# kr4b/pigs

Measured on AMD Instinct MI355X. Metric: sample-points/sec (fwd + 1st + 2nd derivatives, fused), higher is better.
Workload: dtype f32; 1 GPU; c3: 65536 Gaussians x 1024x1024 grid, 1024 rows x 1024 points per GPU, d=2, c=1, kappa=0.5, orders 0-2; gaussians=65536, points_per_gpu=1048576, step=preprocess (cold: nothing reused) + fused forward (orders 0..2)

## Files before the change

pigs_amd/csrc/build_choice.h:

```cpp
#pragma once
#include "plan.h"
#include <stddef.h>
#include <string.h>

namespace pigs {

constexpr uint32_t LISTS_SMALL_TILES = 4096;
constexpr int64_t LATTICE_MIN_POINTS = 1 << 12;
constexpr int64_t COARSE_MIN_POINTS = 1 << 17;
constexpr int64_t STAGE_MIN_POINTS = 1 << 19;
constexpr uint32_t TRUST_MIN_BUILDS = 64;
constexpr float STRIP_MAX_COVER = 64.f;
constexpr int64_t STRIP_MIN_GAUSSIANS = 1024;

struct BuildRequest {
    bool do_samples = false, do_plan = false;
    bool plan_ws_clean = false;
    bool no_lookback = false;
    bool build_lists = true;
    int order = 0;
    bool defer_lists = false, fwd_only = false;
    int64_t N = 0, M = 0;
    int c = 1;
    float q_max = 1.f, q_max_b = 1.f;
};

struct BuildEnv {
    int lattice = -1;
    int lattice_trust = -1;
    int samples_order = 0;
    int gauss_strips = -1;
    int bbox_blocks = -1;
    bool no_ahead = false;
};

struct MemoryAnswer {
    bool coarse = false;
    uint32_t rf = 0, axis = 0;
    bool box_ok = false;
    float box[4] = {0.f, 0.f, 0.f, 0.f};
    bool trust = false;
    bool takes_strips = false;
};

enum BuildKernel : uint32_t {
    K_SAMPLES_BBOX, K_PLAN_ZERO, K_PLAN_COUNT, K_PLAN_SCAN, K_PLAN_SCATTER, K_BINSORT_16, K_BINSORT_1,
    K_LISTS_SMALL,
    K_LISTS
};
struct BuildLaunch {
    BuildKernel kernel;
    uint32_t grid, block, lds;
};
struct BuildChoice {
    bool coarse, no_lattice;
    uint32_t rf_hint, bbox_blocks;
    bool fwd_only, ahead, s_scan_in_scatter, sort_in_count, strips, trusted;
    uint32_t s_blocks;
    float q_max_b;
    BuildLaunch launches[7];
    int n = 0;
    void add(BuildKernel k, uint32_t grid, uint32_t block = 256, uint32_t lds = 0) { launches[n++] = BuildLaunch{k, grid, block, lds}; }
};

inline BuildLaunch list_launch(uint32_t ntiles) {
    const bool small = ntiles <= LISTS_SMALL_TILES && LISTS_TPW != 1;
// ... 135 lines not shown
```

pigs_amd/csrc/build_memory.h:

```cpp
#pragma once
#include <hip/hip_runtime.h>
#include <stdint.h>

namespace pigs {

inline bool current_device(int* dev) {
    if (hipGetDevice(dev) == hipSuccess) return true;
    (void)hipGetLastError();
    return false;
}
inline bool stream_capturing(hipStream_t stream) {
    hipStreamCaptureStatus st = hipStreamCaptureStatusNone;
    if (hipStreamIsCapturing(stream, &st) != hipSuccess) { (void)hipGetLastError(); return false; }
    return st != hipStreamCaptureStatusNone;
}

template <class Key, class State, uint32_t WORDS>
struct BuildMemory {
    struct Slot {
        int device = -1;
        Key key{};
        State st{};
        bool pending = false;
        hipEvent_t ev = nullptr;
        uint32_t* host = nullptr;
        uint64_t stamp = 0;
    };
    void (*landed)(Slot&);
    Slot slots[16];
    uint64_t clock = 0;

    void poll(Slot& s) {
        if (!s.pending) return;
        const hipError_t q = hipEventQuery(s.ev);
        (void)hipGetLastError();
        if (q != hipSuccess) return;
        s.pending = false;
        landed(s);
    }
    Slot* peek(int device, const Key& key) {
        for (auto& s : slots)
            if (s.device == device && s.key == key) return &s;
        return nullptr;
    }
    Slot* find(int device, const Key& key, bool create = false) {
        Slot* lru = nullptr;
        for (auto& s : slots) {
            if (s.device == device && s.key == key) { s.stamp = ++clock; return &s; }
            if (!s.pending && (!lru || s.stamp < lru->stamp)) lru = &s;
        }
        if (!create) return nullptr;
        if (!lru) {
            for (auto& s : slots) {
                poll(s);
                if (!s.pending && (!lru || s.stamp < lru->stamp)) lru = &s;
            }
            if (!lru) return nullptr;
        }
        if (lru->ev && lru->device != device) {
            (void)hipEventDestroy(lru->ev);
            lru->ev = nullptr;
        }
        if (!lru->ev && hipEventCreateWithFlags(&lru->ev, hipEventDisableTiming) != hipSuccess) { lru->ev = nullptr; (void)hipGetLastError(); return nullptr; }
        if (!lru->host && hipHostMalloc((void**)&lru->host, WORDS * sizeof(uint32_t), hipHostMallocPortable) != hipSuccess) { lru->host = nullptr; (void)hipGetLastError(); return nullptr; }
        lru->device = device; lru->key = key; lru->st = State{}; lru->pending = false; lru->stamp = ++clock;
        return lru;
    }
    void request(Slot& s, const void* src, hipStream_t stream) {
        if (hipMemcpyAsync(s.host, src, WORDS * sizeof(uint32_t), hipMemcpyDeviceToHost, stream) == hipSuccess &&
            hipEventRecord(s.ev, stream) == hipSuccess)
            s.pending = true;
        (void)hipGetLastError();
    }
};

}
```

pigs_amd/csrc/plan.hip:

```cpp
#include "pair_math.h"
#include "plan.h"
#include "grid_walk.h"
#include "launch.h"
#include "plan_build.h"
#include "plan_lists.h"
#include "plan_forward.h"
#include "plan_backward.h"
#include "build_choice.h"
#include "build_memory.h"
#include <cstdlib>
#include <cstring>
#include <type_traits>
#include <mutex>
#include <unordered_map>

namespace pigs {

static bool samples_supported(int64_t M) { return M >= 1 && M < (1LL << 31) - 64; }
static bool plan_supported(int64_t N, int64_t M, int c) {
    return samples_supported(M) && N >= 1 && c >= 1 && c <= 2 && N < (1LL << LIST_IDX_BITS);
}

static SamplesView make_samples_view(const SamplesLayout& p, const void* sws) {
    const char* b = (const char*)sws;
// ... 75 lines not shown
    if (coarse) {
        a.scounts = (uint32_t*)(b + s.off_hist);
        a.sagg = (unsigned long long*)(b + s.off_hagg);
        a.sstarts = (uint32_t*)(b + s.off_hstarts);
        a.s_scan_blocks = s.h_scan_blocks;
        a.szero = (uint32_t*)(b + s.off_hagg);
        a.s_zero_words = (uint32_t)((s.off_hstarts - s.off_hagg) / 4);
    } else {
        a.scounts = (uint32_t*)(b + s.off_counts);
        a.sagg = (unsigned long long*)(b + s.off_agg);
        a.sstarts = (uint32_t*)(b + s.off_starts);
        a.s_scan_blocks = s.scan_blocks;
        a.szero = a.scounts;
        a.s_zero_words = (uint32_t)((s.off_starts - s.off_counts) / 4);
    }
}

static int samples_order_setting() {
    const char* e = getenv("PIGS_SAMPLES_ORDER");
    return !e ? 0 : !strcmp(e, "ordered") ? 1 : !strcmp(e, "unordered") ? 2 : 0;
}
static uint32_t lists_product_setting() {
    const char* e = getenv("PIGS_LISTS_PRODUCT");
    return e && e[0] == '0' ? 0u : 1u;
}
static BuildEnv build_env() {
    static const char* const bbox = getenv("PIGS_BBOX_BLOCKS");
    static const bool no_ahead = getenv("PIGS_NO_AHEAD") != nullptr;
    BuildEnv env;
    if (const char* e = getenv("PIGS_LATTICE")) env.lattice = e[0] != '0';
    if (const char* e = getenv("PIGS_LATTICE_TRUST")) env.lattice_trust = e[0] == '0' ? 0 : e[0] == '1' ? 1 : -1;
    env.samples_order = samples_order_setting();
    if (const char* e = getenv("PIGS_GAUSS_STRIPS")) env.gauss_strips = e[0] == '1';
    if (bbox) env.bbox_blocks = atoi(bbox) == 512 ? 512 : 256;
    env.no_ahead = no_ahead;
    return env;
}

struct OrderKey {
    int64_t M;
    bool operator==(const OrderKey& o) const { return M == o.M; }
};
struct PointsKey {
    int64_t N, M;
    bool operator==(const PointsKey& o) const { return N == o.N && M == o.M; }
};
using OrderMemory = BuildMemory<OrderKey, OrderState, ORDER_WORDS>;
using PointsMemory = BuildMemory<PointsKey, PointsState, POINTS_WORDS>;
static void order_landed(OrderMemory::Slot& s) { s.st.absorb(s.host); }
static void points_landed(PointsMemory::Slot& s);
static std::mutex g_memory_mu;
static OrderMemory g_order{order_landed};
static PointsMemory g_points{points_landed};
static void points_landed(PointsMemory::Slot& s) {
    if (s.st.absorb(s.host))
        if (auto* o = g_order.find(s.device, OrderKey{s.key.M})) o->st.turn_around();
}

static MemoryAnswer ask_memories(const BuildRequest& r, const BuildEnv& env, hipStream_t stream) {
    MemoryAnswer m;
    const bool points = strips_asked(r, env);
    int dev = 0;
    if ((!r.do_samples && !points) || !current_device(&dev)) return m;
    const bool cap = stream_capturing(stream);
    std::lock_guard<std::mutex> lock(g_memory_mu);
    if (r.do_samples)
        if (auto* o = g_order.find(dev, OrderKey{r.M})) {
            if (!cap) g_order.poll(*o);
            m.coarse = o->st.coarse; m.rf = o->st.rf; m.axis = o->st.axis;
            if (o->st.box_stable) { m.box_ok = true; memcpy(m.box, o->st.box, sizeof(m.box)); }
            m.trust = !cap && o->st.trusts(env.lattice_trust);
        }
    if (points)
        if (auto* h = g_points.find(dev, PointsKey{r.N, r.M})) {
            if (!cap) g_points.poll(*h);
            m.takes_strips = h->st.takes_strips();
        }
    return m;
}

static void note_order(const SamplesLayout& s, const void* sws, hipStream_t stream, bool trusted) {
    if (!trusted && (s.M < 64 || stream_capturing(stream))) return;
    int dev = 0;
    if (!current_device(&dev)) return;
    std::lock_guard<std::mutex> lock(g_memory_mu);
    auto* o = g_order.find(dev, OrderKey{s.M}, !trusted);
    if (!o) return;
    if (trusted) { ++o->st.trusted; return; }
    const uint32_t nth = o->st.builds++;
    if (o->st.rf != 0u) ++o->st.streak;
    if (!o->pending && o->st.copy_due(nth)) g_order.request(*o, (const char*)sws + s.off_params, stream);
}
static void note_points(const PlanLayout& p, const void* ws, hipStream_t stream, bool trusted = false) {
    int dev = 0;
    if (stream_capturing(stream) || !current_device(&dev)) return;
    std::lock_guard<std::mutex> lock(g_memory_mu);
    auto* h = g_points.find(dev, PointsKey{p.N, p.M}, true);
    if (!h) return;
    const uint32_t nth = h->st.builds++;
    if (!h->pending && h->st.copy_due(nth, trusted))
        g_points.request(*h, &((const PlanParams*)((const char*)ws + p.off_params))->n_points, stream);
}

static bool points_unordered(int64_t M, hipStream_t stream) {
    if (const char* e = getenv("PIGS_STAGE")) return e[0] == '1';
    if (M < STAGE_MIN_POINTS) return false;
    if (getenv("PIGS_SAMPLES_ORDER")) return samples_order_setting() == 2;
    int dev = 0;
    if (!current_device(&dev)) return false;
    const bool cap = stream_capturing(stream);
    std::lock_guard<std::mutex> lock(g_memory_mu);
    auto* o = g_order.peek(dev, OrderKey{M});
    if (!o) return false;
    if (!cap) g_order.poll(*o);
    return o->st.coarse;
}
static bool plan_expects_points(int64_t N, int64_t M, hipStream_t stream) {
    int dev = 0;
    if (!current_device(&dev)) return false;
    const bool cap = stream_capturing(stream);
    std::lock_guard<std::mutex> lock(g_memory_mu);
    auto* h = g_points.find(dev, PointsKey{N, M});
    if (!h) return false;
    if (!cap) g_points.poll(*h);
    return h->st.has_points;
}

int samples_order_hint(int64_t M) {
    int dev = 0;
    if (!current_device(&dev)) return -1;
    std::lock_guard<std::mutex> lock(g_memory_mu);
    auto* o = g_order.find(dev, OrderKey{M});
    if (!o) return -1;
    g_order.poll(*o);
// ... 84 lines not shown
    }
    if (small && strips) hipLaunchKernelGGL((plan_lists_kernel<1, true>), grid, block, 0, stream, la);
    else if (small) hipLaunchKernelGGL((plan_lists_kernel<1, false>), grid, block, 0, stream, la);
    else if (strips) hipLaunchKernelGGL((plan_lists_kernel<LISTS_TPW, true>), grid, block, 0, stream, la);
    else hipLaunchKernelGGL((plan_lists_kernel<LISTS_TPW, false>), grid, block, 0, stream, la);
}

static int run_build(const BuildRequest& r, void* sws, size_t sws_bytes, void* ws, size_t ws_bytes, const void* means,
                     const void* conics, const void* values, const void* samples, hipStream_t stream) {
    if (!samples_supported(r.M)) return PIGS_ERR_UNSUPPORTED;
    const SamplesLayout s = make_samples_layout(r.M);
    if (!sws || sws_bytes < s.total_bytes) return PIGS_ERR_WORKSPACE;
    PlanLayout p{};
    if (r.do_plan) {
        if (!plan_supported(r.N, r.M, r.c)) return PIGS_ERR_UNSUPPORTED;
        if (!(r.q_max > 0.f)) return PIGS_ERR_INVALID;
        p = make_plan_layout(r.N, r.M, r.c);
        if (!ws || ws_bytes < p.total_bytes) return PIGS_ERR_WORKSPACE;
    }
    const BuildEnv env = build_env();
    const MemoryAnswer mem = ask_memories(r, env, stream);
    const BuildChoice b = choose_build(r, s, p, env, mem);
    BuildArgs a{};
    a.do_samples = r.do_samples; a.do_plan = r.do_plan; a.no_lookback = r.no_lookback;
    a.zero_gacc = !r.plan_ws_clean;
    fill_samples_args(a, s, sws, samples, b.coarse);
    if (r.do_plan) fill_plan_args(a, p, ws, r.q_max, b.q_max_b, means, conics, values);
    a.no_lattice = b.no_lattice; a.rf_hint = b.rf_hint; a.bbox_blocks = b.bbox_blocks; a.s_blocks = b.s_blocks;
    a.hint_axis = mem.axis;
    memcpy(a.hint_box, mem.box, sizeof(a.hint_box));
    a.fwd_only = b.fwd_only; a.ahead = b.ahead; a.s_scan_in_scatter = b.s_scan_in_scatter; a.sort_in_count = b.sort_in_count;
    a.strips = b.strips; a.trusted = b.trusted;
    const bool lists = r.do_plan && r.build_lists && !r.defer_lists;
    ListArgs la{};
    if (lists) {
        la = make_list_args(p, s, ws, sws, r.q_max, a.q_max);
        if (b.trusted) {
            la.lattice_broken = &a.params->lattice_broken;
            const float rf = (float)a.rf_hint, rs = (float)(r.M / a.rf_hint);
            la.guard_n[0] = a.hint_axis ? rs : rf; la.guard_n[1] = a.hint_axis ? rf : rs;
            la.guard_e[0] = 16.f * (a.hint_box[2] - a.hint_box[0]) * 1.001f;
            la.guard_e[1] = 16.f * (a.hint_box[3] - a.hint_box[1]) * 1.001f;
        }
    }
    clear_hip_error();
    for (int i = 0; i < b.n; ++i) {
        const BuildLaunch& l = b.launches[i];
        const dim3 grid(l.grid), block(l.block);
        switch (l.kernel) {
            case K_SAMPLES_BBOX: hipLaunchKernelGGL(samples_bbox_kernel, grid, block, l.lds, stream, a); break;
            case K_PLAN_ZERO: hipLaunchKernelGGL(plan_zero_kernel, grid, block, l.lds, stream, a); break;
            case K_PLAN_COUNT: hipLaunchKernelGGL(plan_count_kernel, grid, block, l.lds, stream, a); break;
            case K_PLAN_SCAN: hipLaunchKernelGGL(plan_scan_kernel, grid, block, l.lds, stream, a); break;
            case K_PLAN_SCATTER: hipLaunchKernelGGL(plan_scatter_kernel, grid, block, l.lds, stream, a); break;
            case K_BINSORT_16: hipLaunchKernelGGL(samples_binsort_kernel<16>, grid, block, l.lds, stream, a); break;
            case K_BINSORT_1: hipLaunchKernelGGL(samples_binsort_kernel<1>, grid, block, l.lds, stream, a); break;
            case K_LISTS_SMALL:
            case K_LISTS: launch_lists(l, la, stream, b.strips, b.fwd_only); break;
        }
    }
    const int rc = launch_status();
    if (r.do_plan) defer_set(ws, r.build_lists && r.defer_lists && rc == PIGS_OK, r.q_max, a.q_max);
    if (rc != PIGS_OK) return rc;
    if (lists) note_points(p, ws, stream, b.trusted);
    if (b.trusted || (r.do_samples && r.order == 0)) note_order(s, sws, stream, b.trusted);
    return rc;
}

size_t aggregate_grid_bytes(int64_t N) {
    if (!plan_supported(N, N, 1)) return 0;
    return align_up(make_samples_layout(N).total_bytes, 256) + make_plan_layout(N, N, 1).total_bytes;
}

int aggregate_grid_build(void* ws, size_t ws_bytes, int64_t N, float q_grid, const float* means, const float* conics,
                         hipStream_t stream) {
    if (!plan_supported(N, N, 1)) return PIGS_ERR_UNSUPPORTED;
    if (!ws || ws_bytes < aggregate_grid_bytes(N)) return PIGS_ERR_WORKSPACE;
    const size_t sb = align_up(make_samples_layout(N).total_bytes, 256);
    BuildRequest r;
    r.do_samples = r.do_plan = true; r.build_lists = false;
    r.N = r.M = N; r.c = 1; r.q_max = r.q_max_b = q_grid;
    return run_build(r, ws, sb, (char*)ws + sb, ws_bytes - sb, means, conics, means, means, stream);
}

void aggregate_grid_levels(int64_t N, int64_t* info) {
    const PlanLayout p = make_plan_layout(N, N, 1);
    info[0] = (int64_t)(align_up(make_samples_layout(N).total_bytes, 256) + p.off_params + offsetof(PlanParams, level_mask));
    info[1] = p.L;
}

PlanView aggregate_grid_view(void* ws, int64_t N, float q_grid) {
    const size_t sb = align_up(make_samples_layout(N).total_bytes, 256);
    return make_view(make_plan_layout(N, N, 1), (char*)ws + sb, q_grid);
}

int samples_build(void* sws, size_t sws_bytes, int64_t M, const void* samples, hipStream_t stream) {
    BuildRequest r;
// ... 112 lines not shown
        default: break;
    }
    if constexpr (C == 2) {
        switch (mask) {
            PIGS_CASE(ORDV) PIGS_CASE(ORDC) PIGS_CASE(ORDN)
            default: break;
        }
    }
#undef PIGS_CASE
    if (!done) return PIGS_ERR_UNSUPPORTED;
    hipLaunchKernelGGL((plan_unpermute_kernel<C>), dim3((pv.N + 255) / 256), dim3(256), 0, stream, pv, (float*)a.g_means,
                       (float*)a.g_conics, (float*)a.g_values);
    return launch_status();
}

int plan_forward(void* ws, size_t ws_bytes, const void* sws, size_t sws_bytes, float q_max, const SampleArgs& a,
                 hipStream_t stream) {
    if (!plan_supported(a.N, a.M, a.c)) return PIGS_ERR_UNSUPPORTED;
    const PlanLayout p = make_plan_layout(a.N, a.M, a.c);
    const SamplesLayout s = make_samples_layout(a.M);
    if (!ws || ws_bytes < p.total_bytes || !sws || sws_bytes < s.total_bytes) return PIGS_ERR_WORKSPACE;
    const PlanView pv = make_view(p, ws, q_max);
    const SamplesView sv = make_samples_view(s, sws);
    float* o[4];
    for (int k = 0; k < 4; ++k) o[k] = mask_uses_slot(a.orders_mask, k) ? (float*)a.out[k] : nullptr;
    const int cm = covering_mask_of(a.orders_mask);
    if (a.c != 1 && a.c != 2) return PIGS_ERR_UNSUPPORTED;
    DeferredLists d{};
    ListArgs la{};
    const bool first = defer_take(ws, d);
    if (first) la = make_list_args(p, s, ws, sws, d.q_f, d.q_wide);
    const int rc = a.c == 1 ? plan_forward_c<1>(pv, sv, cm, o, a, stream, first ? &la : nullptr)
                            : plan_forward_c<2>(pv, sv, cm, o, a, stream, first ? &la : nullptr);
    if (first && rc == PIGS_OK) note_points(p, ws, stream);
    return rc;
}

int plan_backward(void* ws, size_t ws_bytes, const void* sws, size_t sws_bytes, float q_max, const SampleArgs& a,
                  hipStream_t stream) {
    if (!plan_supported(a.N, a.M, a.c)) return PIGS_ERR_UNSUPPORTED;
    const PlanLayout p = make_plan_layout(a.N, a.M, a.c);
    const SamplesLayout s = make_samples_layout(a.M);
    if (!ws || ws_bytes < p.total_bytes || !sws || sws_bytes < s.total_bytes) return PIGS_ERR_WORKSPACE;
    const PlanView pv = make_view(p, ws, q_max);
    const SamplesView sv = make_samples_view(s, sws);
    {
        DeferredLists d{};
        if (defer_take(ws, d)) {
            clear_hip_error();
            launch_lists(list_launch(s.ntiles), make_list_args(p, s, ws, sws, d.q_f, d.q_wide), stream);
            const int rc = launch_status();
            if (rc != PIGS_OK) return rc;
            note_points(p, ws, stream);
        }
    }
    const float* g[4];
    for (int k = 0; k < 4; ++k) g[k] = mask_uses_slot(a.orders_mask, k) ? (const float*)a.gout[k] : nullptr;
    const int cm = covering_mask_of(a.orders_mask);
    switch (a.c) {
        case 1: return plan_backward_c<1>(pv, sv, cm, g, a, stream);
        case 2: return plan_backward_c<2>(pv, sv, cm, g, a, stream);
    }
    return PIGS_ERR_UNSUPPORTED;
}

}
```

pigs_amd/csrc/plan_build.h:

```cpp
#pragma once
#include "pair_math.h"
#include "plan.h"
#include "grid_walk.h"
#include <type_traits>

namespace pigs {

struct BuildArgs {
    SampleParams* sparams;
    float4* sboxes;
    float4* slat;
    int no_lattice;
    uint32_t rf_hint;
    uint32_t* scounts;
    unsigned long long* sagg;
    uint32_t* sstarts;
    uint2* skey;
    SPoint* spts;
    const float* samples;
    uint32_t M, scells_cap, s_scan_blocks, s_zero_words;
    uint32_t s_blocks;
    uint32_t* szero;
    int coarse;
    uint32_t cells_per_bin, h_chunk, h_wgs;
// ... 244 lines not shown
#pragma unroll
        for (int k = 0; k < 8; ++k) sh[wave][k] = v[k];
    }
    __syncthreads();
#pragma unroll
    for (int k = 0; k < 8; ++k) {
        float r = sh[0][k];
        for (int w = 1; w < 4; ++w) r = (k & 2) || k >= 4 ? fmaxf(r, sh[w][k]) : fminf(r, sh[w][k]);
        sbox[k] = r;
    }
}
__device__ __forceinline__ bool lattice_compact(const float* sbox, uint32_t rf, uint32_t rs, uint32_t axis) {
    if (rf == 0u) return false;
    const float ex = sbox[2] - sbox[0], ey = sbox[3] - sbox[1];
    const float nx = (float)(axis ? rs : rf), ny = (float)(axis ? rf : rs);
    return 7.f * (sbox[4] + sbox[6]) * nx <= 16.f * ex && 7.f * (sbox[5] + sbox[7]) * ny <= 16.f * ey;
}

struct Run { int start; uint32_t len; bool leader; };
__device__ __forceinline__ Run run_of(uint32_t k, int lane) {
    const uint32_t prev = __shfl_up(k, 1);
    Run r;
    r.leader = lane == 0 || k != prev;
    const uint64_t lm = __ballot(r.leader);
    const uint64_t upto = (2ull << lane) - 1ull;
    r.start = 63 - __builtin_clzll(lm & upto);
    const uint64_t above = lm & ~upto;
    r.len = (uint32_t)((above ? __builtin_ctzll(above) : 64) - lane);
    return r;
}

__device__ __forceinline__ void samples_hist_part(const BuildArgs& a, uint32_t w, const SampleGrid& sg, uint32_t* lh, int lane);

struct GaussLoad { float m[2], c[3]; };
__device__ __forceinline__ void gauss_scatter_one(const BuildArgs& a, uint32_t i, uint32_t pos) {
    float v[2] = {0.f, 0.f};
    for (int k = 0; k < a.c; ++k) v[k] = a.values[(size_t)i * a.c + k];
    a.rec[2 * pos] = make_float4(a.means[2 * i], a.means[2 * i + 1], a.conics[3 * i], a.conics[3 * i + 1]);
    a.rec[2 * pos + 1] = make_float4(a.conics[3 * i + 2], v[0], v[1], 0.f);
    if (i == 0) {
        a.rec[2 * (size_t)a.N] = make_float4(0.f, 0.f, 0.f, 0.f);
        a.rec[2 * (size_t)a.N + 1] = make_float4(0.f, 0.f, 0.f, 0.f);
    }
    {
        const float ca = a.conics[3 * i], cb = a.conics[3 * i + 1], cc = a.conics[3 * i + 2];
        const float k = a.q_max / (ca * cc - cb * cb);
        float hx = sqrtf(k * cc), hy = sqrtf(k * ca);
        if (!(hx < 3.0e38f)) hx = 3.0e38f;
        if (!(hy < 3.0e38f)) hy = 3.0e38f;
        a.gbox[pos] = make_float4(a.means[2 * i], a.means[2 * i + 1], hx * 1.0001f, hy * 1.0001f);
    }
    a.g2o[pos] = i;
}

__device__ __forceinline__ void strip_box(const BuildArgs& a, uint32_t i, bool valid, float mx, float my, float hx, float hy,
                                          const float* box, bool store) {
    __shared__ float4 rowbox[16];
    const float INF = __builtin_huge_valf();
    if (!(hx < 3.0e38f)) hx = INF;
    if (!(hy < 3.0e38f)) hy = INF;
    float x0 = valid ? mx - hx : INF, x1 = valid ? mx + hx : -INF;
    float y0 = valid ? my - hy : INF, y1 = valid ? my + hy : -INF;
    if (valid && !(mx == mx)) { x0 = -INF; x1 = INF; }
    if (valid && !(my == my)) { y0 = -INF; y1 = INF; }
    row_box_dpp(x0, x1, y0, y1);
    const bool first = (threadIdx.x & 15u) == 0u;
    if (first && i < a.N) {
        const uint32_t strip = i / STRIP;
        if (store) a.pbox[strip] = make_float4(x0, y0, x1, y1);
        const float dx = box[2] - box[0], dy = box[3] - box[1];
        const float w = fminf(x1, box[2]) - fmaxf(x0, box[0]), h = fminf(y1, box[3]) - fmaxf(y0, box[1]);
        float cover = (w > 0.f && h > 0.f && dx > 0.f && dy > 0.f) ? (w * h) / (dx * dy) : 0.f;
        if (!(cover == cover)) cover = 1.f;
        a.parea[strip] = cover;
    }
    if (!store) return;
    if (first) rowbox[threadIdx.x >> 4] = make_float4(x0, y0, x1, y1);
    __syncthreads();
    if (threadIdx.x == 0 && i < a.N) {
        float4 b = rowbox[0];
        for (int r = 1; r < 16; ++r) {
            const float4 q = rowbox[r];
            b.x = fminf(b.x, q.x); b.y = fminf(b.y, q.y); b.z = fmaxf(b.z, q.z); b.w = fmaxf(b.w, q.w);
        }
        a.sbox[i / SUPER] = b;
    }
}
__device__ __forceinline__ void gauss_pack_part(const BuildArgs& a, uint32_t i, const float* box, const GaussLoad& ld) {
    const bool valid = i < a.N;
    float hx = 0.f, hy = 0.f;
    if (valid) {
        gauss_scatter_one(a, i, i);
        const float k = a.q_max / (ld.c[0] * ld.c[2] - ld.c[1] * ld.c[1]);
        hx = sqrtf(k * ld.c[2]) * 1.0001f; hy = sqrtf(k * ld.c[0]) * 1.0001f;
    }
    strip_box(a, i, valid, ld.m[0], ld.m[1], hx, hy, box, true);
}
__device__ __forceinline__ GaussLoad gauss_count_load(const BuildArgs& a, uint32_t bid) {
    GaussLoad ld = {{0.f, 0.f}, {0.f, 0.f, 0.f}};
    const uint32_t i = bid * 256 + threadIdx.x;
    if (i < a.N) {
        ld.m[0] = a.means[2 * i]; ld.m[1] = a.means[2 * i + 1];
        ld.c[0] = a.conics[3 * i]; ld.c[1] = a.conics[3 * i + 1]; ld.c[2] = a.conics[3 * i + 2];
    }
    return ld;
}
__device__ __forceinline__ void gauss_count_part(const BuildArgs& a, uint32_t bid, const float* box, const GaussLoad& ld) {
    const int lane = threadIdx.x & 63;
    const uint32_t i = bid * 256 + threadIdx.x;
    const bool valid = i < a.N;
    const float* gm = ld.m;
    const float* gc = ld.c;
    const GaussGrid g = gauss_grid(box, a.G0);
    if (bid == 0 && threadIdx.x == 0) {
        a.params->gg = g;
        a.params->scan_error = 0;
        a.params->q_f = a.q_f;
        a.params->q_b = a.q_b;
        a.params->n_points = 0u;
        a.params->strips = a.strips ? 1u : 0u;
        a.params->points_wanted = 0u;
        a.params->lattice_broken = 0u;
        a.params->fwd_only = a.fwd_only ? 1u : 0u;
        if (a.strips) a.params->level_mask = 0u;
#pragma unroll
        for (int l = 0; l <= PLAN_MAX_LEVELS; ++l) a.params->level_off[l] = a.level_off[l];
    }
    if (a.strips) {
        gauss_pack_part(a, i, box, ld);
        return;
    }
    uint32_t key = 0xffffffffu;
    int l = 0;
    {
        float hx = 0.f, hy = 0.f;
        if (valid) {
// ... 64 lines not shown
                SPoint sp;
                sp.x = p.x; sp.y = p.y; sp.m = i;
                a.spts[__hip_atomic_load(&a.sstarts[kr.x], __ATOMIC_RELAXED, __HIP_MEMORY_SCOPE_AGENT) + kr.y] = sp;
            }
        }
    }
}

__global__ __launch_bounds__(256) void plan_count_kernel(BuildArgs a) {
    __shared__ float shb[4][8];
    __shared__ uint32_t lh[SAMPLES_COARSE_BINS];
    __shared__ uint32_t scan_sh[4], scan_sh2[4];
    const int lane = threadIdx.x & 63;
    const uint32_t shift = a.ahead && !a.strips ? a.scan_blocks : 0u;
    if (blockIdx.x < shift) {
        scan_block<false>(a, true, blockIdx.x, scan_sh, scan_sh2);
        return;
    }
    const uint32_t bid = blockIdx.x - shift, nb = gridDim.x - shift;
    const uint32_t gblocks = a.do_plan && !a.ahead ? (a.N + 255) / 256 : 0;
    const bool gpart = bid < gblocks;
    float2 pt[4];
    uint32_t i0 = ((bid - gblocks) * 4 + (threadIdx.x >> 6)) * 256 + lane;
    const bool looked = a.do_samples && !a.trusted;
    const uint32_t lat_rf = looked ? a.sparams->lat_cand[0] : 0u;
    const uint32_t lat_axis = looked ? a.sparams->lat_cand[1] : 0u;
    auto load_points = [&]() {
#pragma unroll
        for (int k = 0; k < 4; ++k) {
            const uint32_t i = i0 + 64 * k;
            pt[k] = i < a.M ? ((const float2*)a.samples)[i] : make_float2(0.f, 0.f);
        }
    };
    GaussLoad gld = {{0.f, 0.f}, {0.f, 0.f, 0.f}};
    if (gpart) gld = gauss_count_load(a, bid);
    else if (!a.coarse && lat_rf == 0u) load_points();
    float sbox[8] = {0.f, 0.f, 0.f, 0.f, 0.f, 0.f, 0.f, 0.f};
    bool lattice = false;
    if (a.trusted) {
#pragma unroll
        for (int k = 0; k < 4; ++k) sbox[k] = a.hint_box[k];
        if (bid == 0 && threadIdx.x == 0) {
            SampleParams* sp = a.sparams;
#pragma unroll
            for (int k = 0; k < 4; ++k) sp->box[k] = sbox[k];
            sp->sg = sample_grid(sbox, a.M, a.scells_cap);
            sp->scan_error = 0;
            sp->order_stat[0] = 0u; sp->order_stat[1] = 0u;
            sp->lat_cand[0] = a.rf_hint; sp->lat_cand[1] = a.hint_axis;
            sp->lat[0] = a.rf_hint; sp->lat[1] = a.M / a.rf_hint;
            sp->src = (uint64_t)(uintptr_t)a.samples;
        }
        gauss_count_part(a, bid, sbox, gld);
        return;
    }
    if (a.do_samples) {
        reduce_boxes(a.sboxes, a.slat, a.bbox_blocks, sbox, shb);
        lattice = lattice_compact(sbox, lat_rf, lat_rf ? a.M / lat_rf : 0u, lat_axis);
    } else {
#pragma unroll
        for (int k = 0; k < 4; ++k) sbox[k] = a.sparams->box[k];
    }
    const SampleGrid sg = sample_grid(sbox, a.M, a.scells_cap);
    if (bid == gblocks && threadIdx.x == 0 && a.do_samples) {
#pragma unroll
        for (int k = 0; k < 4; ++k) a.sparams->box[k] = sbox[k];
        a.sparams->sg = sg;
// ... 448 lines not shown
```

pigs_amd/csrc/plan_lists.h:

```cpp
#pragma once
#include "plan_build.h"

#ifndef PIGS_LISTS_PRODUCT
#define PIGS_LISTS_PRODUCT 1
#endif

namespace pigs {

constexpr int SURV_CAP = 128;
template <int TPW>
struct ListsLds {
    TravLds trav;
    float4 sa[SURV_CAP];
    float4 sb[SURV_CAP];
    float4 gbox[TPW * 4];
    float4 tbox[TPW];
    uint32_t sel[SURV_CAP];
};
static_assert(4 * sizeof(ListsLds<4>) <= 32768, "five workgroups of the list launch per CU");
struct ListArgs {
    PlanView pv;
    SamplesView sv;
    uint32_t* hdr;
    uint32_t* tlist;
    uint32_t* glist;
    uint32_t* ptiles;
    uint32_t* n_points;
    uint32_t* points_wanted;
    float q_f;
    const float* parea;
    float* strip_cover;
    uint32_t product;
    uint32_t* lattice_broken;
    float guard_n[2], guard_e[2];
};

template <int TPW, bool STRIPS = false, bool FWD_ONLY = false, bool PRODUCT = true>
__device__ __forceinline__ void build_block_lists(const ListArgs& a, ListsLds<TPW>& lds, uint32_t tile0, int lane) {
    const PlanView& pv = a.pv;
    const uint32_t ntiles = a.sv.ntiles;
    constexpr bool strips = STRIPS;
    GaussGrid gg{};
    uint32_t level_mask = 0u, loff = 0u;
    if constexpr (STRIPS) {
        gg.inv_s0 = pv.params->gg.inv_s0;
    } else {
        gg = pv.params->gg;
        level_mask = pv.params->level_mask;
        loff = pv.params->level_off[lane < PLAN_MAX_LEVELS ? lane : 0];
    }
    const float INF = __builtin_huge_valf();
    SPoint sp[TPW];
    bool valid[TPW];
    const PointOrder po = point_order(a.sv);
#pragma unroll
    for (int t = 0; t < TPW; ++t) {
        const uint32_t m = (tile0 + (uint32_t)t) * TILE_POINTS + (uint32_t)lane;
        valid[t] = m < a.sv.M;
        sp[t] = SPoint{0.f, 0.f, 0u};
        if (tile0 + (uint32_t)t < ntiles) sp[t] = tile_point(a.sv, po, tile0 + (uint32_t)t, (uint32_t)lane);
    }
    float bx0 = INF, bx1 = -INF, by0 = INF, by1 = -INF;
    float gx0[TPW], gx1[TPW], gy0[TPW], gy1[TPW];
    uint32_t has[TPW];
#pragma unroll
    for (int t = 0; t < TPW; ++t) {
        float x0 = valid[t] ? sp[t].x : INF, x1 = valid[t] ? sp[t].x : -INF;
        float y0 = valid[t] ? sp[t].y : INF, y1 = valid[t] ? sp[t].y : -INF;
        row_box_dpp(x0, x1, y0, y1);
        if ((lane & 15) == 0) lds.gbox[t * 4 + (lane >> 4)] = make_float4(x0, y0, x1, y1);
        bx0 = fminf(bx0, x0); bx1 = fmaxf(bx1, x1); by0 = fminf(by0, y0); by1 = fmaxf(by1, y1);
        gx0[t] = x0; gx1[t] = x1; gy0[t] = y0; gy1[t] = y1;
        const uint64_t hm = __ballot(x0 <= x1);
        has[t] = (uint32_t)(hm & 1ull) | (uint32_t)(hm >> 15 & 2ull) | (uint32_t)(hm >> 30 & 4ull) | (uint32_t)(hm >> 45 & 8ull);
    }
    wave_box_from_rows_dpp(bx0, bx1, by0, by1);
    wave_lds_fence();
    if (lane < TPW) {
        const float4 g0 = lds.gbox[lane * 4], g1 = lds.gbox[lane * 4 + 1], g2 = lds.gbox[lane * 4 + 2], g3 = lds.gbox[lane * 4 + 3];
        lds.tbox[lane] = make_float4(fminf(fminf(g0.x, g1.x), fminf(g2.x, g3.x)), fminf(fminf(g0.y, g1.y), fminf(g2.y, g3.y)),
                                     fmaxf(fmaxf(g0.z, g1.z), fmaxf(g2.z, g3.z)), fmaxf(fmaxf(g0.w, g1.w), fmaxf(g2.w, g3.w)));
    }
    wave_lds_fence();
    constexpr bool CAN_PRODUCT = PRODUCT && PIGS_LISTS_PRODUCT != 0 && (TPW == 1 || TPW == 4);
// ... 1 lines not shown
    bool product = false;
    if constexpr (CAN_PRODUCT) {
        auto same = [](float u, float v) { return __builtin_bit_cast(uint32_t, u) == __builtin_bit_cast(uint32_t, v); };
        bool ok = a.product != 0u;
#pragma unroll
        for (int t = 0; t < TPW; ++t) ok = ok && has[t] == 15u;
        if (__builtin_amdgcn_readfirstlane((int)ok)) {
            if constexpr (TPW == 4) {
                ok = ok && same(gx0[0], gx0[1]) && same(gx1[0], gx1[1]) && same(gx0[2], gx0[3]) && same(gx1[2], gx1[3]);
                ok = ok && same(gy0[0], gy0[2]) && same(gy1[0], gy1[2]) && same(gy0[1], gy0[3]) && same(gy1[1], gy1[3]);
            }
#pragma unroll
            for (int h = 0; h < (TPW == 4 ? 2 : 1); ++h) {
                const int tc = 2 * h, tr = h;
                ok = ok && same(gx0[tc], __shfl_xor(gx0[tc], 32)) && same(gx1[tc], __shfl_xor(gx1[tc], 32));
                ok = ok && same(gy0[tr], __shfl_xor(gy0[tr], 16)) && same(gy1[tr], __shfl_xor(gy1[tr], 16));
            }
            product = __ballot(ok) == ~0ull;
        }
    }

    const uint32_t cap = pv.list_cap;
    auto walk_candidates = [&]() -> float {
        float e = 0.f;
        if (lane < pv.L) {
            const float cells = (float)(pv.G0 >> lane) * (float)(pv.G0 >> lane);
            e = 9.f * (float)(pv.starts[pv.level_off[lane + 1]] - pv.starts[pv.level_off[lane]]) / cells;
        }
#pragma unroll
        for (int o = 1; o < 16; o <<= 1) e += __shfl_xor(e, o);
        return __shfl(e, 0);
    };
    if (strips && (bx1 - bx0) * gg.inv_s0 * ((by1 - by0) * gg.inv_s0) > POINTS_MODE_BLOCK_CELLS) {
        if (lane == 0) atomicAdd(a.points_wanted, 1u);
    }
    if (!strips && (bx1 - bx0) * gg.inv_s0 * ((by1 - by0) * gg.inv_s0) > POINTS_MODE_BLOCK_CELLS && walk_candidates() <= 4.f * (float)cap) {
        for (int t = 0; t < TPW; ++t) {
            if (tile0 + (uint32_t)t >= ntiles) break;
            if (lane < TILE_HDR_WORDS)
                a.hdr[(size_t)(tile0 + (uint32_t)t) * TILE_HDR_WORDS + lane] = lane == 0 ? (TILE_MODE_POINTS << TILE_MODE_SHIFT) : 0u;
            if (lane == 0) a.ptiles[atomicAdd(a.n_points, 1u)] = tile0 + (uint32_t)t;
        }
        return;
    }
    uint32_t n[TPW], ng[TPW][4];
    bool overflow[TPW], goverflow[TPW];
#pragma unroll
    for (int t = 0; t < TPW; ++t) {
        n[t] = 0; overflow[t] = false; goverflow[t] = false;
#pragma unroll
        for (int g = 0; g < 4; ++g) ng[t][g] = 0;
    }
    int sn = 0;
    auto append = [&](int t, uint32_t j, uint32_t gm, uint32_t gf) __attribute__((always_inline)) {
        uint32_t* tl = a.tlist + (size_t)(tile0 + (uint32_t)t) * cap;
        uint32_t* gl = a.glist + (size_t)(tile0 + (uint32_t)t) * 4 * cap;
        if constexpr (!FWD_ONLY) {
            const uint64_t km = __ballot(gm != 0u);
            const uint32_t cnt = (uint32_t)__builtin_popcountll(km);
            if (n[t] + cnt <= cap) {
                if (gm != 0u) tl[n[t] + (uint32_t)lanes_below(km)] = j | (gm << LIST_WIDE_SHIFT) | (gf << LIST_NARROW_SHIFT);
            } else {
                overflow[t] = true;
            }
            n[t] += cnt;
        }
#pragma unroll
        for (int g = 0; g < 4; ++g) {
            const uint64_t mg = __ballot(gf >> g & 1u);
            const uint32_t cg = (uint32_t)__builtin_popcountll(mg);
            if (ng[t][g] + cg <= cap) {
                if (gf >> g & 1u) gl[g * cap + ng[t][g] + (uint32_t)lanes_below(mg)] = j;
            } else {
                goverflow[t] = true;
// ... 89 lines not shown
        if (product) flush_product();
        else flush_general();
    };
    auto walk_rect = [&](float x0, float y0, float x1, float y1, bool walk, auto&& rows, auto&& batch) __attribute__((always_inline)) {
        if constexpr (STRIPS) traverse_strips(pv, x0, y0, x1, y1, lane, lds.trav, walk, rows, batch);
        else traverse(pv, gg, level_mask, loff, x0, y0, x1, y1, lane, lds.trav, walk, rows, batch);
    };
    walk_rect(bx0, by0, bx1, by1, true,
             [](int, uint32_t, uint32_t) {},
             [&](const float4 A, const float4 B, uint64_t mask, uint32_t j) __attribute__((always_inline)) {
        const int add = __builtin_popcountll(mask);
        if (sn + add > SURV_CAP) flush();
        if (mask >> lane & 1ull) {
            const Ellipse e = ellipse_of(A, B.x);
            const int k = sn + lanes_below(mask);
            lds.sa[k] = A;
            lds.sb[k] = make_float4(B.x, e.nb_c, e.nb_a, __builtin_bit_cast(float, j));
        }
        sn += add;
    });
    if (sn > 0) flush();

    const bool two_cuts = !FWD_ONLY && pv.q_max > a.q_f;
    bool any_rare = false;
    bool rebuild[TPW];
    const bool guard = a.lattice_broken != nullptr;
#pragma unroll
    for (int t = 0; t < TPW; ++t) {
        rebuild[t] = false;
        if (tile0 + (uint32_t)t >= ntiles) { overflow[t] = false; continue; }
        if (guard) {
            const float4 tb = lds.tbox[t];
            const float wx = tb.z - tb.x, wy = tb.w - tb.y;
            if (!(wx * a.guard_n[0] <= a.guard_e[0] && wy * a.guard_n[1] <= a.guard_e[1]) && lane == 0) *a.lattice_broken = 1u;
        }
        const bool tl_over = FWD_ONLY ? goverflow[t] : overflow[t];
        overflow[t] = tl_over && goverflow[t];
        rebuild[t] = tl_over && !goverflow[t] && two_cuts;
        uint32_t longest = ng[t][0] > ng[t][1] ? ng[t][0] : ng[t][1];
        longest = ng[t][2] > longest ? ng[t][2] : longest;
        longest = ng[t][3] > longest ? ng[t][3] : longest;
        if (longest > POINTS_MODE_MIN_LIST) {
            const float4 tb = lds.tbox[t];
            const float wx = tb.z - tb.x, wy = tb.w - tb.y;
            if (strips && wx * gg.inv_s0 * (wy * gg.inv_s0) > POINTS_MODE_MIN_CELLS) {
                if (lane == 0) atomicAdd(a.points_wanted, 1u);
            }
            if (!strips && wx * gg.inv_s0 * (wy * gg.inv_s0) > POINTS_MODE_MIN_CELLS && walk_candidates() <= 4.f * (float)(longest < cap ? longest : cap)) {
                overflow[t] = false; rebuild[t] = false;
                if (lane < 5)
                    a.hdr[(size_t)(tile0 + (uint32_t)t) * TILE_HDR_WORDS + lane] = lane == 0 ? (TILE_MODE_POINTS << TILE_MODE_SHIFT) : 0u;
                if (lane == 0) a.ptiles[atomicAdd(a.n_points, 1u)] = tile0 + (uint32_t)t;
                continue;
            }
        }
        any_rare |= overflow[t] || rebuild[t];
        if (!overflow[t] && !rebuild[t] && lane < TILE_HDR_WORDS) {
            const bool fits = n[t] <= cap;
            uint32_t w = 0;
            if (lane == 0) w = fits ? ((n[t] & TILE_COUNT_MASK) | (TILE_MODE_LIST << TILE_MODE_SHIFT)) : (TILE_MODE_GROUPS << TILE_MODE_SHIFT);
#pragma unroll
            for (int g = 0; g < 4; ++g)
                if (lane == 1 + g) w = ng[t][g];
            if (lane < 5) a.hdr[(size_t)(tile0 + (uint32_t)t) * TILE_HDR_WORDS + lane] = w;
        }
    }
    if (!any_rare) return;
    for (int t = 0; t < TPW; ++t) {
        const bool mine_rebuild = __builtin_amdgcn_readfirstlane((int)(t == 0   ? rebuild[0]
                                                                       : t == 1 ? rebuild[TPW > 1 ? 1 : 0]
                                                                       : t == 2 ? rebuild[TPW > 2 ? 2 : 0]
                                                                                : rebuild[TPW > 3 ? 3 : 0])) != 0;
        bool mine = __builtin_amdgcn_readfirstlane((int)(t == 0   ? overflow[0]
                                                         : t == 1 ? overflow[TPW > 1 ? 1 : 0]
                                                         : t == 2 ? overflow[TPW > 2 ? 2 : 0]
                                                                  : overflow[TPW > 3 ? 3 : 0])) != 0;
        if (!mine && !mine_rebuild) continue;
        float4 gb[4];
#pragma unroll
        for (int g = 0; g < 4; ++g) gb[g] = lds.gbox[t * 4 + g];
        const float4 tb = lds.tbox[t];
        const float tx0 = tb.x, ty0 = tb.y, tx1 = tb.z, ty1 = tb.w;
        uint32_t* tl = a.tlist + (size_t)(tile0 + (uint32_t)t) * cap;
        if (mine_rebuild) {
            uint32_t* gl = a.glist + (size_t)(tile0 + (uint32_t)t) * 4 * cap;
// ... 4 lines not shown
                     [&](const float4 A, const float4 B, uint64_t mask, uint32_t j) __attribute__((always_inline)) {
                const bool have = mask >> lane & 1ull;
                const Ellipse e = ellipse_of(A, B.x);
#pragma unroll
                for (int g = 0; g < 4; ++g) {
                    const bool hit = have && gb[g].x <= gb[g].z &&
                                     !(ellipse_min_q_rect(e, gb[g].x, gb[g].y, gb[g].z, gb[g].w) > pv.q_max);
                    const uint64_t mg = __ballot(hit);
                    const uint32_t cg = (uint32_t)__builtin_popcountll(mg);
                    if (ngw[g] + cg <= cap) {
                        if (hit) gl[g * cap + ngw[g] + (uint32_t)lanes_below(mg)] = j;
                    } else {
                        gover = true;
                    }
                    ngw[g] += cg;
                }
            });
            if (!gover) {
                if (lane < 5) {
                    uint32_t w = 0;
                    if (lane == 0) w = TILE_MODE_GROUPS << TILE_MODE_SHIFT;
#pragma unroll
                    for (int g = 0; g < 4; ++g)
                        if (lane == 1 + g) w = ngw[g];
                    a.hdr[(size_t)(tile0 + (uint32_t)t) * TILE_HDR_WORDS + lane] = w;
                }
                continue;
            }
            mine = true;
        }
        if (!strips && (tx1 - tx0) * gg.inv_s0 * ((ty1 - ty0) * gg.inv_s0) > POINTS_MODE_MIN_CELLS && walk_candidates() <= 4.f * (float)cap) {
            if (lane < 5)
                a.hdr[(size_t)(tile0 + (uint32_t)t) * TILE_HDR_WORDS + lane] = lane == 0 ? (TILE_MODE_POINTS << TILE_MODE_SHIFT) : 0u;
            if (lane == 0) a.ptiles[atomicAdd(a.n_points, 1u)] = tile0 + (uint32_t)t;
            continue;
        }
        uint32_t nr = 0;
        bool fits = true;
        walk_rect(tx0, ty0, tx1, ty1, false,
                 [&](int nrow, uint32_t jb, uint32_t len) {
            const bool keep = lane < nrow && len > 0;
            const uint64_t km = __ballot(keep);
            const uint32_t cnt = (uint32_t)__builtin_popcountll(km);
            if (2 * (nr + cnt) <= cap) {
                if (keep) {
                    const uint32_t p = 2 * (nr + (uint32_t)lanes_below(km));
                    tl[p] = jb; tl[p + 1] = len;
                }
            } else {
                fits = false;
            }
            nr += cnt;
        },
                 [](const float4, const float4, uint64_t, uint32_t) {});
        if (!fits && lane == 0) { tl[0] = 0; tl[1] = pv.N; }
        const uint32_t cnt = fits ? nr : 1u;
        if (lane < 5)
            a.hdr[(size_t)(tile0 + (uint32_t)t) * TILE_HDR_WORDS + lane] = lane == 0 ? (cnt | (TILE_MODE_RANGES << TILE_MODE_SHIFT)) : 0u;
    }
}

template <int TPW>
__device__ __forceinline__ uint32_t lists_tile0(int wave) {
    return (xcd_block_chunk<PIGS_XCD_CHUNK / TPW>(gridDim.x) * 4 + (uint32_t)wave) * TPW;
}
__device__ __forceinline__ void lists_strip_cover(const ListArgs& a) {
    __shared__ float cover_sh[4];
    if (blockIdx.x != 0) return;
    const uint32_t ns = (a.pv.N + STRIP - 1u) / STRIP;
    float sum = 0.f;
    for (uint32_t k = threadIdx.x; k < ns; k += 256u) sum += a.parea[k];
#pragma unroll
    for (int o = 32; o > 0; o >>= 1) sum += __shfl_xor(sum, o);
    if ((threadIdx.x & 63u) == 0u) cover_sh[threadIdx.x >> 6] = sum;
    __syncthreads();
    if (threadIdx.x == 0) a.strip_cover[0] = cover_sh[0] + cover_sh[1] + cover_sh[2] + cover_sh[3];
}

template <int TPW, bool STRIPS, bool FWD_ONLY = false>
__global__ __launch_bounds__(256, 5) void plan_lists_kernel(ListArgs a) {
    __shared__ ListsLds<TPW> lds_all[4];
    const int lane = threadIdx.x & 63;
    const int wave = __builtin_amdgcn_readfirstlane(threadIdx.x >> 6);
    lists_strip_cover(a);
    const uint32_t tile0 = lists_tile0<TPW>(wave);
    if (tile0 >= a.sv.ntiles) return;
    build_block_lists<TPW, STRIPS, FWD_ONLY>(a, lds_all[wave], tile0, lane);
}

}
```

Before: 23.12 billion sample-points/s.

## Write build statistics to mapped host memory and skip strip-area measurement when unneeded

```diff
diff --git a/pigs_amd/csrc/build_choice.h b/pigs_amd/csrc/build_choice.h
--- a/pigs_amd/csrc/build_choice.h
+++ b/pigs_amd/csrc/build_choice.h
@@ -32,6 +32,7 @@
     int gauss_strips = -1;
     int bbox_blocks = -1;
     bool no_ahead = false;
+    bool stats_home = true;
 };
 
 struct MemoryAnswer {
diff --git a/pigs_amd/csrc/build_memory.h b/pigs_amd/csrc/build_memory.h
--- a/pigs_amd/csrc/build_memory.h
+++ b/pigs_amd/csrc/build_memory.h
@@ -22,8 +22,10 @@
         Key key{};
         State st{};
         bool pending = false;
+        bool recorded = false;
         hipEvent_t ev = nullptr;
         uint32_t* host = nullptr;
+        uint32_t* dev = nullptr;
         uint64_t stamp = 0;
     };
     void (*landed)(Slot&);
@@ -31,7 +33,7 @@
     uint64_t clock = 0;
 
     void poll(Slot& s) {
-        if (!s.pending) return;
+        if (!s.pending || !s.recorded) return;
         const hipError_t q = hipEventQuery(s.ev);
         (void)hipGetLastError();
         if (q != hipSuccess) return;
@@ -60,16 +62,28 @@
         if (lru->ev && lru->device != device) {
             (void)hipEventDestroy(lru->ev);
             lru->ev = nullptr;
+            lru->dev = nullptr;
         }
         if (!lru->ev && hipEventCreateWithFlags(&lru->ev, hipEventDisableTiming) != hipSuccess) { lru->ev = nullptr; (void)hipGetLastError(); return nullptr; }
-        if (!lru->host && hipHostMalloc((void**)&lru->host, WORDS * sizeof(uint32_t), hipHostMallocPortable) != hipSuccess) { lru->host = nullptr; (void)hipGetLastError(); return nullptr; }
-        lru->device = device; lru->key = key; lru->st = State{}; lru->pending = false; lru->stamp = ++clock;
+        if (!lru->host && hipHostMalloc((void**)&lru->host, WORDS * sizeof(uint32_t), hipHostMallocMapped | hipHostMallocPortable) != hipSuccess) { lru->host = nullptr; (void)hipGetLastError(); return nullptr; }
+        if (!lru->dev && hipHostGetDevicePointer((void**)&lru->dev, lru->host, 0) != hipSuccess) { lru->dev = nullptr; (void)hipGetLastError(); return nullptr; }
+        lru->device = device; lru->key = key; lru->st = State{}; lru->pending = lru->recorded = false; lru->stamp = ++clock;
         return lru;
     }
+    void reserve(Slot& s) { s.pending = true; s.recorded = false; }
+    void release(Slot& s) { s.pending = false; s.recorded = false; }
+    uint32_t* home(Slot& s) {
+        for (uint32_t k = 0; k < WORDS; ++k) s.host[k] = 0u;
+        return s.dev;
+    }
+    void sent(Slot& s, hipStream_t stream) {
+        s.recorded = hipEventRecord(s.ev, stream) == hipSuccess;
+        if (!s.recorded) s.pending = false;
+        (void)hipGetLastError();
+    }
     void request(Slot& s, const void* src, hipStream_t stream) {
-        if (hipMemcpyAsync(s.host, src, WORDS * sizeof(uint32_t), hipMemcpyDeviceToHost, stream) == hipSuccess &&
-            hipEventRecord(s.ev, stream) == hipSuccess)
-            s.pending = true;
+        s.pending = s.recorded = hipMemcpyAsync(s.host, src, WORDS * sizeof(uint32_t), hipMemcpyDeviceToHost, stream) == hipSuccess &&
+                                 hipEventRecord(s.ev, stream) == hipSuccess;
         (void)hipGetLastError();
     }
 };
diff --git a/pigs_amd/csrc/plan.hip b/pigs_amd/csrc/plan.hip
--- a/pigs_amd/csrc/plan.hip
+++ b/pigs_amd/csrc/plan.hip
@@ -131,6 +131,7 @@
     if (const char* e = getenv("PIGS_LATTICE_TRUST")) env.lattice_trust = e[0] == '0' ? 0 : e[0] == '1' ? 1 : -1;
     env.samples_order = samples_order_setting();
     if (const char* e = getenv("PIGS_GAUSS_STRIPS")) env.gauss_strips = e[0] == '1';
+    if (const char* e = getenv("PIGS_STATS_HOME")) env.stats_home = e[0] != '0';
     if (bbox) env.bbox_blocks = atoi(bbox) == 512 ? 512 : 256;
     env.no_ahead = no_ahead;
     return env;
@@ -190,15 +191,32 @@
     if (o->st.rf != 0u) ++o->st.streak;
     if (!o->pending && o->st.copy_due(nth)) g_order.request(*o, (const char*)sws + s.off_params, stream);
 }
-static void note_points(const PlanLayout& p, const void* ws, hipStream_t stream, bool trusted = false) {
+static PointsMemory::Slot* points_due(const PlanLayout& p, hipStream_t stream, bool trusted) {
     int dev = 0;
-    if (stream_capturing(stream) || !current_device(&dev)) return;
+    if (stream_capturing(stream) || !current_device(&dev)) return nullptr;
     std::lock_guard<std::mutex> lock(g_memory_mu);
     auto* h = g_points.find(dev, PointsKey{p.N, p.M}, true);
-    if (!h) return;
+    if (!h) return nullptr;
     const uint32_t nth = h->st.builds++;
-    if (!h->pending && h->st.copy_due(nth, trusted))
-        g_points.request(*h, &((const PlanParams*)((const char*)ws + p.off_params))->n_points, stream);
+    if (h->pending || !h->st.copy_due(nth, trusted)) return nullptr;
+    g_points.reserve(*h);
+    return h;
+}
+static uint32_t* points_home(PointsMemory::Slot& h, bool strips) {
+    std::lock_guard<std::mutex> lock(g_memory_mu);
+    uint32_t* home = g_points.home(h);
+    h.host[HOME_STRIPS] = strips ? 1u : 0u;
+    return home;
+}
+static void note_points(PointsMemory::Slot& h, bool ok, const uint32_t* home, const PlanLayout& p, const void* ws, hipStream_t stream) {
+    std::lock_guard<std::mutex> lock(g_memory_mu);
+    if (!ok) g_points.release(h);
+    else if (home) g_points.sent(h, stream);
+    else g_points.request(h, &((const PlanParams*)((const char*)ws + p.off_params))->n_points, stream);
+}
+
+static void note_deferred_points(const PlanLayout& p, const void* ws, hipStream_t stream) {
+    if (PointsMemory::Slot* due = points_due(p, stream, false)) note_points(*due, true, nullptr, p, ws, stream);
 }
 
 static bool points_unordered(int64_t M, hipStream_t stream) {
@@ -349,9 +367,15 @@
     a.fwd_only = b.fwd_only; a.ahead = b.ahead; a.s_scan_in_scatter = b.s_scan_in_scatter; a.sort_in_count = b.sort_in_count;
     a.strips = b.strips; a.trusted = b.trusted;
     const bool lists = r.do_plan && r.build_lists && !r.defer_lists;
+    PointsMemory::Slot* due = lists ? points_due(p, stream, b.trusted) : nullptr;
+    const bool deferred = r.do_plan && r.build_lists && r.defer_lists;
+    const bool measure = deferred || (lists && (due || !env.stats_home));
+    if (!measure) a.parea = nullptr;
     ListArgs la{};
     if (lists) {
         la = make_list_args(p, s, ws, sws, r.q_max, a.q_max);
+        if (!measure) la.parea = nullptr;
+        if (due && env.stats_home) la.home = points_home(*due, b.strips);
         if (b.trusted) {
             la.lattice_broken = &a.params->lattice_broken;
             const float rf = (float)a.rf_hint, rs = (float)(r.M / a.rf_hint);
@@ -378,8 +402,8 @@
     }
     const int rc = launch_status();
     if (r.do_plan) defer_set(ws, r.build_lists && r.defer_lists && rc == PIGS_OK, r.q_max, a.q_max);
+    if (due) note_points(*due, rc == PIGS_OK, la.home, p, ws, stream);
     if (rc != PIGS_OK) return rc;
-    if (lists) note_points(p, ws, stream, b.trusted);
     if (b.trusted || (r.do_samples && r.order == 0)) note_order(s, sws, stream, b.trusted);
     return rc;
 }
@@ -558,7 +582,7 @@
     if (first) la = make_list_args(p, s, ws, sws, d.q_f, d.q_wide);
     const int rc = a.c == 1 ? plan_forward_c<1>(pv, sv, cm, o, a, stream, first ? &la : nullptr)
                             : plan_forward_c<2>(pv, sv, cm, o, a, stream, first ? &la : nullptr);
-    if (first && rc == PIGS_OK) note_points(p, ws, stream);
+    if (first && rc == PIGS_OK) note_deferred_points(p, ws, stream);
     return rc;
 }
 
@@ -577,7 +601,7 @@
             launch_lists(list_launch(s.ntiles), make_list_args(p, s, ws, sws, d.q_f, d.q_wide), stream);
             const int rc = launch_status();
             if (rc != PIGS_OK) return rc;
-            note_points(p, ws, stream);
+            note_deferred_points(p, ws, stream);
         }
     }
     const float* g[4];
diff --git a/pigs_amd/csrc/plan_build.h b/pigs_amd/csrc/plan_build.h
--- a/pigs_amd/csrc/plan_build.h
+++ b/pigs_amd/csrc/plan_build.h
@@ -300,7 +300,7 @@
 
 __device__ __forceinline__ void samples_hist_part(const BuildArgs& a, uint32_t w, const SampleGrid& sg, uint32_t* lh, int lane);
 
-struct GaussLoad { float m[2], c[3]; };
+struct GaussLoad { float m[2], c[3], v[2]; };
 __device__ __forceinline__ void gauss_scatter_one(const BuildArgs& a, uint32_t i, uint32_t pos) {
     float v[2] = {0.f, 0.f};
     for (int k = 0; k < a.c; ++k) v[k] = a.values[(size_t)i * a.c + k];
@@ -336,6 +336,9 @@
     if (first && i < a.N) {
         const uint32_t strip = i / STRIP;
         if (store) a.pbox[strip] = make_float4(x0, y0, x1, y1);
+    }
+    if (first && i < a.N && a.parea) {
+        const uint32_t strip = i / STRIP;
         const float dx = box[2] - box[0], dy = box[3] - box[1];
         const float w = fminf(x1, box[2]) - fmaxf(x0, box[0]), h = fminf(y1, box[3]) - fmaxf(y0, box[1]);
         float cover = (w > 0.f && h > 0.f && dx > 0.f && dy > 0.f) ? (w * h) / (dx * dy) : 0.f;
@@ -358,18 +361,29 @@
     const bool valid = i < a.N;
     float hx = 0.f, hy = 0.f;
     if (valid) {
-        gauss_scatter_one(a, i, i);
+        a.rec[2 * i] = make_float4(ld.m[0], ld.m[1], ld.c[0], ld.c[1]);
+        a.rec[2 * i + 1] = make_float4(ld.c[2], ld.v[0], ld.v[1], 0.f);
+        if (i == 0) {
+            a.rec[2 * (size_t)a.N] = make_float4(0.f, 0.f, 0.f, 0.f);
+            a.rec[2 * (size_t)a.N + 1] = make_float4(0.f, 0.f, 0.f, 0.f);
+        }
+        a.g2o[i] = i;
         const float k = a.q_max / (ld.c[0] * ld.c[2] - ld.c[1] * ld.c[1]);
         hx = sqrtf(k * ld.c[2]) * 1.0001f; hy = sqrtf(k * ld.c[0]) * 1.0001f;
     }
     strip_box(a, i, valid, ld.m[0], ld.m[1], hx, hy, box, true);
 }
 __device__ __forceinline__ GaussLoad gauss_count_load(const BuildArgs& a, uint32_t bid) {
-    GaussLoad ld = {{0.f, 0.f}, {0.f, 0.f, 0.f}};
+    GaussLoad ld = {{0.f, 0.f}, {0.f, 0.f, 0.f}, {0.f, 0.f}};
     const uint32_t i = bid * 256 + threadIdx.x;
     if (i < a.N) {
         ld.m[0] = a.means[2 * i]; ld.m[1] = a.means[2 * i + 1];
         ld.c[0] = a.conics[3 * i]; ld.c[1] = a.conics[3 * i + 1]; ld.c[2] = a.conics[3 * i + 2];
+        if (a.strips) {
+#pragma unroll
+            for (int k = 0; k < 2; ++k)
+                if (k < a.c) ld.v[k] = a.values[(size_t)i * a.c + k];
+        }
     }
     return ld;
 }
@@ -500,7 +514,7 @@
             pt[k] = i < a.M ? ((const float2*)a.samples)[i] : make_float2(0.f, 0.f);
         }
     };
-    GaussLoad gld = {{0.f, 0.f}, {0.f, 0.f, 0.f}};
+    GaussLoad gld = {{0.f, 0.f}, {0.f, 0.f, 0.f}, {0.f, 0.f}};
     if (gpart) gld = gauss_count_load(a, bid);
     else if (!a.coarse && lat_rf == 0u) load_points();
     float sbox[8] = {0.f, 0.f, 0.f, 0.f, 0.f, 0.f, 0.f, 0.f};
diff --git a/pigs_amd/csrc/plan_lists.h b/pigs_amd/csrc/plan_lists.h
--- a/pigs_amd/csrc/plan_lists.h
+++ b/pigs_amd/csrc/plan_lists.h
@@ -30,10 +30,16 @@
     float q_f;
     const float* parea;
     float* strip_cover;
+    uint32_t* home;
     uint32_t product;
     uint32_t* lattice_broken;
     float guard_n[2], guard_e[2];
 };
+
+__device__ __forceinline__ void stats_home(uint32_t* home, uint32_t word, uint32_t v) {
+    __hip_atomic_store(home + word, v, __ATOMIC_RELAXED, __HIP_MEMORY_SCOPE_SYSTEM);
+}
+constexpr uint32_t HOME_N_POINTS = 0, HOME_STRIP_COVER = 1, HOME_STRIPS = 2, HOME_POINTS_WANTED = 3, HOME_LATTICE_BROKEN = 4;
 
 template <int TPW, bool STRIPS = false, bool FWD_ONLY = false, bool PRODUCT = true>
 __device__ __forceinline__ void build_block_lists(const ListArgs& a, ListsLds<TPW>& lds, uint32_t tile0, int lane) {
@@ -50,6 +56,18 @@
         loff = pv.params->level_off[lane < PLAN_MAX_LEVELS ? lane : 0];
     }
     const float INF = __builtin_huge_valf();
+    auto queue_points_tile = [&](uint32_t tile) {
+        const uint32_t k = atomicAdd(a.n_points, 1u);
+        a.ptiles[k] = tile;
+        if (k == 0u && a.home) stats_home(a.home, HOME_N_POINTS, 1u);
+    };
+    auto note_points_wanted = [&]() {
+        if (a.home) {
+            if (atomicAdd(a.points_wanted, 1u) == 0u) stats_home(a.home, HOME_POINTS_WANTED, 1u);
+        } else {
+            atomicAdd(a.points_wanted, 1u);
+        }
+    };
     SPoint sp[TPW];
     bool valid[TPW];
     const PointOrder po = point_order(a.sv);
@@ -117,14 +135,14 @@
         return __shfl(e, 0);
     };
     if (strips && (bx1 - bx0) * gg.inv_s0 * ((by1 - by0) * gg.inv_s0) > POINTS_MODE_BLOCK_CELLS) {
-        if (lane == 0) atomicAdd(a.points_wanted, 1u);
+        if (lane == 0) note_points_wanted();
     }
     if (!strips && (bx1 - bx0) * gg.inv_s0 * ((by1 - by0) * gg.inv_s0) > POINTS_MODE_BLOCK_CELLS && walk_candidates() <= 4.f * (float)cap) {
         for (int t = 0; t < TPW; ++t) {
             if (tile0 + (uint32_t)t >= ntiles) break;
             if (lane < TILE_HDR_WORDS)
                 a.hdr[(size_t)(tile0 + (uint32_t)t) * TILE_HDR_WORDS + lane] = lane == 0 ? (TILE_MODE_POINTS << TILE_MODE_SHIFT) : 0u;
-            if (lane == 0) a.ptiles[atomicAdd(a.n_points, 1u)] = tile0 + (uint32_t)t;
+            if (lane == 0) queue_points_tile(tile0 + (uint32_t)t);
         }
         return;
     }
@@ -280,7 +298,10 @@
         if (guard) {
             const float4 tb = lds.tbox[t];
             const float wx = tb.z - tb.x, wy = tb.w - tb.y;
-            if (!(wx * a.guard_n[0] <= a.guard_e[0] && wy * a.guard_n[1] <= a.guard_e[1]) && lane == 0) *a.lattice_broken = 1u;
+            if (!(wx * a.guard_n[0] <= a.guard_e[0] && wy * a.guard_n[1] <= a.guard_e[1]) && lane == 0) {
+                *a.lattice_broken = 1u;
+                if (a.home) stats_home(a.home, HOME_LATTICE_BROKEN, 1u);
+            }
         }
         const bool tl_over = FWD_ONLY ? goverflow[t] : overflow[t];
         overflow[t] = tl_over && goverflow[t];
@@ -292,13 +313,13 @@
             const float4 tb = lds.tbox[t];
             const float wx = tb.z - tb.x, wy = tb.w - tb.y;
             if (strips && wx * gg.inv_s0 * (wy * gg.inv_s0) > POINTS_MODE_MIN_CELLS) {
-                if (lane == 0) atomicAdd(a.points_wanted, 1u);
+                if (lane == 0) note_points_wanted();
             }
             if (!strips && wx * gg.inv_s0 * (wy * gg.inv_s0) > POINTS_MODE_MIN_CELLS && walk_candidates() <= 4.f * (float)(longest < cap ? longest : cap)) {
                 overflow[t] = false; rebuild[t] = false;
                 if (lane < 5)
                     a.hdr[(size_t)(tile0 + (uint32_t)t) * TILE_HDR_WORDS + lane] = lane == 0 ? (TILE_MODE_POINTS << TILE_MODE_SHIFT) : 0u;
-                if (lane == 0) a.ptiles[atomicAdd(a.n_points, 1u)] = tile0 + (uint32_t)t;
+                if (lane == 0) queue_points_tile(tile0 + (uint32_t)t);
                 continue;
             }
         }
@@ -369,7 +390,7 @@
         if (!strips && (tx1 - tx0) * gg.inv_s0 * ((ty1 - ty0) * gg.inv_s0) > POINTS_MODE_MIN_CELLS && walk_candidates() <= 4.f * (float)cap) {
             if (lane < 5)
                 a.hdr[(size_t)(tile0 + (uint32_t)t) * TILE_HDR_WORDS + lane] = lane == 0 ? (TILE_MODE_POINTS << TILE_MODE_SHIFT) : 0u;
-            if (lane == 0) a.ptiles[atomicAdd(a.n_points, 1u)] = tile0 + (uint32_t)t;
+            if (lane == 0) queue_points_tile(tile0 + (uint32_t)t);
             continue;
         }
         uint32_t nr = 0;
@@ -403,7 +424,7 @@
 }
 __device__ __forceinline__ void lists_strip_cover(const ListArgs& a) {
     __shared__ float cover_sh[4];
-    if (blockIdx.x != 0) return;
+    if (blockIdx.x != 0 || a.parea == nullptr) return;
     const uint32_t ns = (a.pv.N + STRIP - 1u) / STRIP;
     float sum = 0.f;
     for (uint32_t k = threadIdx.x; k < ns; k += 256u) sum += a.parea[k];
@@ -411,7 +432,12 @@
     for (int o = 32; o > 0; o >>= 1) sum += __shfl_xor(sum, o);
     if ((threadIdx.x & 63u) == 0u) cover_sh[threadIdx.x >> 6] = sum;
     __syncthreads();
-    if (threadIdx.x == 0) a.strip_cover[0] = cover_sh[0] + cover_sh[1] + cover_sh[2] + cover_sh[3];
+    if (threadIdx.x == 0) {
+        const float cover = cover_sh[0] + cover_sh[1] + cover_sh[2] + cover_sh[3];
+        a.strip_cover[0] = cover;
+        const uint32_t w = __builtin_bit_cast(uint32_t, cover);
+        if (a.home && w != 0u) stats_home(a.home, HOME_STRIP_COVER, w);
+    }
 }
 
 template <int TPW, bool STRIPS, bool FWD_ONLY = false>
```

New measurement: 23.43 billion sample-points/s, median of 6. 1.4% higher.
